# MoayedHajiAli/ElasticDiffusion-official

Hardware: AMD Instinct MI355X
Metric: images/sec at 50 steps (SDXL 2048x1024) (higher is better)
Workload: dtype fp16

## Files before the change

### elasticdiffusion_official_amd/_hip.py

```python
import ctypes
import os
import subprocess

import torch

PKG_DIR = os.path.dirname(os.path.abspath(__file__))
ROOT_DIR = os.path.dirname(PKG_DIR)
SOURCES = [os.path.join(PKG_DIR, "csrc", n) for n in ("elastic_kernels.hip", "unet_kernels.hip", "attention_kernels.hip", "gemm_kernels.hip", "vae_kernels.hip",
                                                       "canny_kernels.hip", "resize_kernels.hip", "mask_kernels.hip", "lora_kernels.hip", "pca_kernels.hip")]
SRC = SOURCES[0]
INCLUDE = os.path.join(ROOT_DIR, "include")
SO_PATH = os.path.join(PKG_DIR, "libelastic_hip.so")
ABI_VERSION = 13

HIPCC_FLAGS = ["--offload-arch=gfx950", "-O3", "-std=c++17", "-ffp-contract=off", "-fPIC", "-shared"]

_i32p = ctypes.POINTER(ctypes.c_int32)
_vp, _i, _f, _i64 = ctypes.c_void_p, ctypes.c_int, ctypes.c_float, ctypes.c_int64

SIGNATURES = {
    "ed_version": [],
    "ed_error_string": [_i],
    "ed_gather_views": [_vp, _vp, _i, _i, _i, _i, _i, _vp, _vp, _i, _i, _i, _i, _i, _i, _i, _vp, _f, _vp],
    "ed_scatter_centres": [_vp, _i, _vp, _i, _i, _i, _i, _i, _i, _i, _vp, _vp, _vp, _vp, _vp],
    "ed_pick_assemble": [_vp, _vp, _vp, _vp, _vp, _vp, _i, _vp, _i, _i, _i, _i, _i, _i, _i, _i, _i, _i, _i, _vp],
    "ed_unpad_direction": [_vp, _i, _vp, _vp, _i, _i, _i, _i, _i, _i, _i, _i, _i, _vp],
    "ed_fill_directions": [_vp, _vp, _vp, _vp, _vp, _vp, _vp, _vp, _vp, _vp, _i, _i, _i, _i, _i, _i, _i, _vp],
    "ed_cfg_ddim_step": [_vp, _vp, _vp, _vp, _vp, _f, _f, _f, _f, _f, _i64, _vp],
    "ed_undo_step": [_vp, _vp, _vp, _vp, _i, _i64, _vp],
    "ed_rrg_update": [_vp, _vp, _vp, _vp, _vp, _vp, _vp, _vp, _f, _f, _f, _f, _f, _i, _i, _i, _i, _i, _i, _vp],
    "ed_gather2d": [_vp, _i, _vp, _i, _i, _i, _i, _vp, _vp, _vp, _i, _i, _i, _vp],
    "ed_tile_gather_pad": [_vp, _vp, _i, _i, _i, _i, _i, _vp, _vp, _i, _i, _f, _vp],
    "ed_tile_accumulate_normalise": [_vp, _i, _vp, _i, _i, _i, _i, _i, _i, _vp, _vp, _vp, _vp, _vp],
    "ed_geglu": [_vp, _vp, _i, _i64, _i, _vp],
    "ed_groupnorm": [_vp, _vp, _vp, _vp, _vp, _vp, _vp, _i, _i, _i, _i, _i, _f, _i, _i, _vp],
    "ed_groupnorm_workspace": [_i, _i, _i, _i],
    "ed_bias_residual_add": [_vp, _vp, _vp, _vp, _vp, _i, _i, _i, _i, _i, _vp],
    "ed_add_layernorm": [_vp, _vp, _vp, _vp, _vp, _vp, _i, _i64, _i, _f, _vp],
    "ed_tokens_add_nchw": [_vp, _vp, _vp, _i, _i, _i, _i, _vp],
    "ed_layernorm": [_vp, _vp, _vp, _vp, _i, _i64, _i, _f, _vp],
    "ed_layernorm_s32": [_vp, _vp, _vp, _vp, _i, _i64, _i, _f, _vp],
    "ed_add_layernorm_s32": [_vp, _vp, _vp, _vp, _vp, _vp, _i, _i64, _i, _f, _vp],
    "ed_groupnorm_nhwc_s32": [_vp, _vp, _vp, _vp, _vp, _i, _i, _i, _i, _i, _f, _i, _vp],
    "ed_groupnorm_nhwc": [_vp, _vp, _vp, _vp, _vp, _vp, _vp, _i, _i, _i, _i, _i, _f, _i, _vp],
    "ed_groupnorm_nhwc_workspace": [_i, _i, _i, _i],
    "ed_groupnorm_nhwc_cat": [_vp, _vp, _vp, _vp, _vp, _vp, _i, _i, _i, _i, _i, _i, _f, _i, _vp],
    "ed_assemble_rows": [_vp, _i, _i, _i, _i, _vp, _vp, _vp, _vp, _vp, _vp, _i, _i, _i, _i, _i, _i, _i, _vp, _vp, _vp, _vp,
                         _i, _i, _i, _i, _i, _i, _i, _i, _vp],
# ... 66 lines not shown
    "ed_assemble_rows_n": [_vp, _i, _i, _i, _i, _vp, _vp, _vp, _vp, _vp, _vp, _i, _i, _i, _i, _i, _i, _i, _vp, _vp, _vp, _vp,
                           _i, _i, _i, _i, _i, _i, _i, _i, _vp, _i, _vp, _i, _vp],
    "ed_region_blend": [_vp, _vp, _vp, _i, _i, _i64, _vp],
    "ed_phase_epilogue_rg": [_vp, _vp, _i, _vp, _vp, _vp, _vp, _vp, _vp, _vp, _vp, _vp, _vp, _vp, _vp, _vp, _vp, _vp, _vp,
                             _vp, _vp, _vp, _vp, _i, _i, _i, _i, _i, _i, _i, _i, _i, _i, _i, _i, _i, _i, _f, _f, _f, _f, _f,
                             _f, _f, _f, _f, _i, _vp, _vp, _f, _f, _vp, _i, _vp, _i, _vp],
    "ed_phase_moments_rg": [_vp, _vp, _i, _vp, _vp, _vp, _vp, _vp, _vp, _vp, _vp, _vp, _vp, _vp, _vp, _vp, _vp, _i, _i, _i, _i,
                            _i, _i, _i, _i, _i, _i, _i, _i, _i, _i, _f, _vp, _i, _vp],
    "ed_score_pca_workspace": [_i, _i64],
    "ed_score_pca_fit": [_vp, _i, _i, _i, _i, _i, _vp, _vp, _vp, _vp, _vp, _vp],
    "ed_score_pca_map": [_vp, _i, _i, _i, _i, _vp, _vp, _vp, _vp],
    "ed_groupnorm_nhwc_f32_weighted": [_vp, _vp, _vp, _vp, _vp, _i, _i, _i, _i, _i, _f, _i, _i, _vp, _vp, _vp],
    "ed_groupnorm_f32_weighted": [_vp, _vp, _vp, _vp, _vp, _i, _i, _i, _i, _i, _f, _i, _vp, _vp, _vp],
    "ed_softmax_rows_bias": [_vp, _i64, _i64, _f, _vp, _vp],
    "ed_control_residuals": [_vp, _i, _i, _vp, _i64, _vp],
    "ed_flash_attention_ipn": [_vp, _vp, _vp, _vp, _i, _i, _i, _i, _i, _i, _vp, _i, _i64, _i64, _i64, _i64, _i64, _i64, _i64, _i64, _f,
                               _vp, _vp],
    "ed_flash_attention_ipm": [_vp, _vp, _vp, _vp, _i, _i, _i, _i, _i, _i, _vp, _i, _i64, _i64, _i64, _i64, _i64, _i64, _i64, _i64, _f,
                               _vp, _vp, _i64, _i64, _vp],
    "ed_ip_mask_rows": [_vp, _i, _i, _i, _i, _vp, _vp, _vp, _i, _i, _i, _i, _i, _vp, _vp, _i, _i, _i, _i, _i, _i, _i, _i, _vp, _vp],
}

_LIB = None


def build_library(force=False, verbose=False):
    deps = SOURCES + [os.path.join(INCLUDE, "elastic_hip.h")]
    if not force and os.path.isfile(SO_PATH) and os.path.getmtime(SO_PATH) >= max(os.path.getmtime(d) for d in deps):
        return SO_PATH
    import tempfile
    flags = [f for f in HIPCC_FLAGS if f != "-shared"]
    with tempfile.TemporaryDirectory(prefix="ed_build_") as tmp:
        objs = [os.path.join(tmp, os.path.basename(src) + ".o") for src in SOURCES]
        cmds = [["hipcc", *flags, "-I", INCLUDE, "-c", src, "-o", obj] for src, obj in zip(SOURCES, objs)]
        if verbose:
            for c in cmds:
                print(" ".join(c))
        procs = [subprocess.Popen(c) for c in cmds]
        codes = [p.wait() for p in procs]
        if any(codes):
            raise subprocess.CalledProcessError(next(c for c in codes if c), cmds[[bool(c) for c in codes].index(True)])
        link = ["hipcc", "--offload-arch=gfx950", "-fPIC", "-shared", *objs, "-o", SO_PATH + ".tmp"]
        if verbose:
            print(" ".join(link))
        subprocess.run(link, check=True)
        os.replace(SO_PATH + ".tmp", SO_PATH)
    return SO_PATH


def lib():
    global _LIB
    if _LIB is None:
        if not os.path.isfile(SO_PATH):
            raise RuntimeError(
                f"{SO_PATH} is missing: the HIP kernels are the product path and there is no CPU fallback. "
                "Build it with `python -c 'import __graft_entry__ as g; g.build()'`.")
        L = ctypes.CDLL(SO_PATH)
        for name, argtypes in SIGNATURES.items():
            fn = getattr(L, name)
            fn.argtypes = argtypes
            fn.restype = (ctypes.c_char_p if name == "ed_error_string" else
                          ctypes.c_int64 if name.endswith("_workspace") else ctypes.c_int)
        if L.ed_version() != ABI_VERSION:
            raise RuntimeError(f"libelastic_hip.so ABI {L.ed_version()} != expected {ABI_VERSION}; rebuild")
        _LIB = L
    return _LIB

# ... 6 lines not shown
```

### elasticdiffusion_official_amd/csrc/attention_kernels.hip

```cpp
#include <hip/hip_runtime.h>
#include <stdint.h>

#include "elastic_hip.h"

namespace {

constexpr int D = 64;
constexpr int QB = 128;
constexpr int KT = 64;
constexpr int K_LD = 72;
constexpr int V_LD_TR = 96;
constexpr int V_LD_T = 68;

typedef float f32x16 __attribute__((ext_vector_type(16)));
typedef float f32x8 __attribute__((ext_vector_type(8)));
typedef short s16x4 __attribute__((ext_vector_type(4)));
typedef short s16x8 __attribute__((ext_vector_type(8)));
typedef __bf16 bf16x8 __attribute__((ext_vector_type(8)));
typedef _Float16 f16x8 __attribute__((ext_vector_type(8)));

struct alignas(16) Vec16 { uint32_t w[4]; };
struct alignas(8) Vec8 { uint32_t w[2]; };

struct BF {
  typedef bf16x8 v8;
  static __device__ __forceinline__ f32x16 mfma(v8 a, v8 b, f32x16 c) {
    return __builtin_amdgcn_mfma_f32_32x32x16_bf16(a, b, c, 0, 0, 0);
  }
  static __device__ __forceinline__ v8 pack(f32x8 p) { return __builtin_convertvector(p, v8); }
};
struct HF {
  typedef f16x8 v8;
  static __device__ __forceinline__ f32x16 mfma(v8 a, v8 b, f32x16 c) {
    return __builtin_amdgcn_mfma_f32_32x32x16_f16(a, b, c, 0, 0, 0);
// ... 388 lines not shown
    pf[g] = T::pack(pv);
    asm volatile("" : "+v"(pf[g]));
  }
}

template <typename T>
__device__ __forceinline__ void resoftmax_tile(const uint16_t* kt, int ln, int hi, const typename T::v8 (&qf)[4],
                                               f32x16 (&s)[2], float sl, SoftmaxRun& r, typename T::v8 (&pf)[4]) {
  qk_tile<T>(kt, ln, hi, qf, s);
  float mx = s[0][0];
#pragma unroll
  for (int j = 1; j < 16; ++j) mx = fmaxf(mx, s[0][j]);
#pragma unroll
  for (int j = 0; j < 16; ++j) mx = fmaxf(mx, s[1][j]);
  mx = fmaxf(mx, __shfl_xor(mx, 32, 64));
  const float use = fmaxf(r.mb, mx * sl);
  r.alpha = __builtin_amdgcn_exp2f(r.mb - use);
  r.mb = use;
  float psum = 0.f;
#pragma unroll
  for (int g = 0; g < 4; ++g) {
    f32x8 pv;
#pragma unroll
    for (int j = 0; j < 8; ++j) {
      const int f = 8 * g + j;
      pv[j] = __builtin_amdgcn_exp2f(__builtin_fmaf(s[f >> 4][f & 15], sl, -use));
      psum += pv[j];
    }
    pf[g] = T::pack(pv);
  }
  r.psum = psum;
}

template <typename T, bool HAS_PV, bool HAS_NEXT, bool LAZY, bool EXP2, int DEPTH, class Filler>
__device__ __forceinline__ void pipe_region(Filler&& filler, const uint16_t* k_next, const uint16_t* v_prev, int lane, int ln, int hi,
                                            const typename T::v8 (&qf)[4], f32x16 (&s_cur)[2], f32x16 (&s_next)[2],
                                            const typename T::v8 (&p_prev)[4], typename T::v8 (&p_cur)[4],
                                            f32x16 (&o)[2], float sl, SoftmaxRun& run, const f32x16& negm) {
  constexpr int NQK = HAS_NEXT ? 8 : 0, N = NQK + (HAS_PV ? 8 : 0);
  auto fetch = [&](int i) -> Vec16 {
    if (i < NQK) return *reinterpret_cast<const Vec16*>(&k_next[(32 * (i & 1) + ln) * K_LD + 16 * (i >> 1) + 8 * hi]);
    const int j = i - NQK;
    return v_frag_tr(v_prev, lane, hi, j >> 1, j & 1);
  };
  if (HAS_NEXT && !EXP2) {
#pragma unroll
    for (int i = 0; i < 16; ++i) s_next[0][i] = s_next[1][i] = 0.f;
  }
  Vec16 ring[DEPTH + 1];
#pragma unroll
  for (int r = 0; r <= DEPTH; ++r) ring[r] = Vec16{{0u, 0u, 0u, 0u}};
#pragma unroll
  for (int r = 0; r < DEPTH; ++r)
    if (r < N) ring[r] = fetch(r);
#pragma unroll
  for (int i = 0; i < 16; ++i) {
    if (i < N) {
      if (i + DEPTH < N) ring[(i + DEPTH) % (DEPTH + 1)] = fetch(i + DEPTH);
      const Vec16 a_cur = ring[i % (DEPTH + 1)];
      if (i < NQK) {
        if (EXP2 && i < 2) s_next[i & 1] = T::mfma(as_v8<typename T::v8>(a_cur), qf[0], negm);
        else s_next[i & 1] = T::mfma(as_v8<typename T::v8>(a_cur), qf[i >> 1], s_next[i & 1]);
        asm volatile("" : "+v"(s_next[i & 1]));
      } else {
        const int j = i - NQK;
        o[j & 1] = T::mfma(as_v8<typename T::v8>(a_cur), p_prev[j >> 1], o[j & 1]);
        asm volatile("" : "+v"(o[j & 1]));
      }
    }
    if (LAZY) softmax_slice_lazy<T, EXP2>(i, s_cur, sl, run, p_cur);
    else softmax_slice<T>(i, s_cur, sl, run, p_cur);
    filler(i);
    __builtin_amdgcn_sched_barrier(0);
  }
}

template <typename T, bool LAZY, bool EXP2 = false, int DEPTH = 1, int WAVES = 4>
__global__ void __launch_bounds__(64 * WAVES, 2)
k_flash_attn_pipe(const Params p) {
  static_assert(LAZY || !EXP2, "the exponent-domain variant is built on the lazy-maximum loop");
  static_assert(WAVES == 4 || WAVES == 8, "4 or 8 waves per workgroup");
  constexpr int NK = LAZY ? 3 : 2;
  constexpr int NST = 8 / WAVES;
  __shared__ SmemPipe<NK> sm;
  const int tid = threadIdx.x;
  const int lane = tid & 63, wave = tid >> 6;
  const int ln = lane & 31, hi = lane >> 5;
  int bh, qblk;
  {
    const int id = blockIdx.x, per = 8 * p.nqb, grp = id / per, r = id - grp * per;
    if ((grp + 1) * 8 <= p.BH) {
      bh = grp * 8 + (r & 7);
      qblk = r >> 3;
    } else {
      bh = grp * 8 + r / p.nqb;
      qblk = r % p.nqb;
    }
  }
  const int b = bh / p.H, h = bh - b * p.H;
  const uint16_t* qg = p.q + b * p.q_sb + h * D;
  const uint16_t* kg = p.k + b * p.k_sb + h * D;
  const uint16_t* vg = p.v + b * p.v_sb + h * D;
  uint16_t* og = p.o + b * p.o_sb + h * D;

  const int q_row = qblk * (32 * WAVES) + wave * 32 + ln;
  typename T::v8 qf[4];
#pragma unroll
  for (int ks = 0; ks < 4; ++ks) qf[ks] = as_v8<typename T::v8>(load_row16(qg, p.q_sn, q_row, p.Nq, 16 * ks + 8 * hi));

  const BufRsrc k_rs = make_rsrc(kg, ((int64_t)(p.Nk - 1) * p.k_sn + D) * 2);
  const BufRsrc v_rs = make_rsrc(vg, ((int64_t)(p.Nk - 1) * p.v_sn + D) * 2);
  const int st_row = tid >> 3, st_col = (tid & 7) * 8;
  const uint32_t k_off = (uint32_t)(((int64_t)st_row * p.k_sn + st_col) * 2), k_half = (uint32_t)(32 * p.k_sn * 2);
  const uint32_t v_off = (uint32_t)(((int64_t)st_row * p.v_sn + st_col) * 2), v_half = (uint32_t)(32 * p.v_sn * 2);
  Vec16 kreg[NST], vreg[NST];
  auto load_k = [&](int t) {
    const uint32_t base = k_off + (uint32_t)t * 2u * k_half;
#pragma unroll
    for (int i = 0; i < NST; ++i) kreg[i] = buf_load16(k_rs, base + i * k_half, 0);
  };
  auto load_v = [&](int t) {
    const uint32_t base = v_off + (uint32_t)t * 2u * v_half;
#pragma unroll
    for (int i = 0; i < NST; ++i) vreg[i] = buf_load16(v_rs, base + i * v_half, 0);
  };
  auto write_k = [&](int buf) {
#pragma unroll
    for (int i = 0; i < NST; ++i) *reinterpret_cast<Vec16*>(&sm.k[buf][(st_row + 32 * i) * K_LD + st_col]) = kreg[i];
  };
  auto write_v = [&](int buf) {
#pragma unroll
    for (int i = 0; i < NST; ++i) *reinterpret_cast<Vec16*>(&sm.v[buf][(st_row + 32 * i) * V_LD_TR + st_col]) = vreg[i];
  };

  f32x16 oacc[2];
#pragma unroll
  for (int i = 0; i < 16; ++i) oacc[0][i] = oacc[1][i] = 0.f;
  SoftmaxRun run;
  run.mb = -INFINITY, run.l = 0.f, run.mx = 0.f, run.use = 0.f, run.alpha = 1.f, run.psum = 0.f;
  const float sl = EXP2 ? 1.0f : p.scale_log2e;
  const int n_tiles = (p.Nk + KT - 1) / KT, n_full = p.Nk / KT;
  f32x16 negm;
#pragma unroll
  for (int i = 0; i < 16; ++i) negm[i] = 0.f;

  load_k(0);
  load_v(0);
  Vec16 k1reg[NST];
#pragma unroll
  for (int i = 0; i < NST; ++i) k1reg[i] = buf_load16(k_rs, k_off + 2u * k_half + i * k_half, 0);
  write_k(0);
  write_v(0);
#pragma unroll
  for (int i = 0; i < NST; ++i) *reinterpret_cast<Vec16*>(&sm.k[1][(st_row + 32 * i) * K_LD + st_col]) = k1reg[i];
  __syncthreads();

  f32x16 sA[2], sB[2];
  typename T::v8 pA[4], pB[4];
  int vb_prev = 2, vb_cur = 0, vb_next = 1;
  int kb_cur = 0, kb_next = 1, kb_write = NK == 3 ? 2 : 0;

  auto iter = [&](auto has_pv, auto has_next, int t, f32x16 (&s_cur)[2], f32x16 (&s_next)[2],
                  typename T::v8 (&p_prev)[4], typename T::v8 (&p_cur)[4]) {
    const uint32_t kbase = k_off + (uint32_t)(t + 2) * 2u * k_half, vbase = v_off + (uint32_t)(t + 1) * 2u * v_half;
    uint16_t* const kdst = sm.k[kb_write];
    uint16_t* const vdst = sm.v[vb_next];
    auto filler = [&](int i) {
      if (i < NST) kreg[i] = buf_load16(k_rs, kbase + i * k_half, 0);
      else if (i < 2 * NST) vreg[i - NST] = buf_load16(v_rs, vbase + (i - NST) * v_half, 0);
      else if (i >= 11 && i < 11 + NST) *reinterpret_cast<Vec16*>(&kdst[(st_row + 32 * (i - 11)) * K_LD + st_col]) = kreg[i - 11];
      else if (i >= 11 + NST && i < 11 + 2 * NST)
        *reinterpret_cast<Vec16*>(&vdst[(st_row + 32 * (i - 11 - NST)) * V_LD_TR + st_col]) = vreg[i - 11 - NST];
    };
    constexpr bool lazy = LAZY && (EXP2 || decltype(has_pv)::value);
    pipe_region<T, decltype(has_pv)::value, decltype(has_next)::value, lazy, EXP2, DEPTH>(filler, sm.k[kb_next], sm.v[vb_prev], lane, ln,
                                                                                          hi, qf, s_cur, s_next, p_prev, p_cur,
                                                                                          oacc, sl, run, negm);
    if (lazy) {
      run.alpha = 1.0f;
      if (__any(!(run.psum <= RESCALE_SUM_MAX))) {
        const float mb_old = run.mb;
        resoftmax_tile<T>(sm.k[kb_cur], ln, hi, qf, s_cur, sl, run, p_cur);
        if (EXP2) {
          const float d = run.mb - mb_old;
          if (decltype(has_next)::value) {
#pragma unroll
            for (int i = 0; i < 16; ++i) s_next[0][i] -= d, s_next[1][i] -= d;
          }
#pragma unroll
          for (int i = 0; i < 16; ++i) negm[i] = -run.mb;
          asm volatile("" : "+v"(negm));
        }
      }
      run.l = __builtin_fmaf(run.l, run.alpha, run.psum);
    }
    if (__any(run.alpha != 1.0f)) {
#pragma unroll
      for (int i = 0; i < 16; ++i) {
        oacc[0][i] *= run.alpha;
        oacc[1][i] *= run.alpha;
      }
    }
    const int tmp = vb_prev;
    vb_prev = vb_cur, vb_cur = vb_next, vb_next = tmp;
    const int ktmp = kb_cur;
    kb_cur = kb_next, kb_next = kb_write, kb_write = NK == 3 ? ktmp : kb_cur;
    __syncthreads();
  };

  if (n_full > 0) {
    qk_tile<T>(sm.k[0], ln, hi, qf, sA);
    if (EXP2) {
      float mx = sA[0][0];
#pragma unroll
      for (int j = 1; j < 16; ++j) mx = fmaxf(mx, sA[0][j]);
#pragma unroll
      for (int j = 0; j < 16; ++j) mx = fmaxf(mx, sA[1][j]);
      mx = fmaxf(mx, __shfl_xor(mx, 32, 64));
      run.mb = mx;
#pragma unroll
      for (int i = 0; i < 16; ++i) sA[0][i] -= mx, sA[1][i] -= mx, negm[i] = -mx;
      asm volatile("" : "+v"(negm));
    }
    __syncthreads();
    if (n_full == 1) {
      iter(False{}, False{}, 0, sA, sB, pB, pA);
    } else {
      iter(False{}, True{}, 0, sA, sB, pB, pA);
      int t = 1;
      for (; t + 2 < n_full; t += 2) {
        iter(True{}, True{}, t, sB, sA, pA, pB);
        iter(True{}, True{}, t + 1, sA, sB, pB, pA);
      }
      if (n_full - t == 2) {
        iter(True{}, True{}, t, sB, sA, pA, pB);
        iter(True{}, False{}, t + 1, sA, sB, pB, pA);
      } else {
        iter(True{}, False{}, t, sB, sA, pA, pB);
      }
    }
    if ((n_full - 1) & 1) pv_tile<T>(sm.v[vb_prev], lane, hi, pB, oacc);
    else pv_tile<T>(sm.v[vb_prev], lane, hi, pA, oacc);
  }

  if (n_tiles > n_full) {
    f32x16 s[2];
    qk_tile<T>(sm.k[kb_cur], ln, hi, qf, s);
#pragma unroll
    for (int kb = 0; kb < 2; ++kb)
#pragma unroll
      for (int r = 0; r < 16; ++r)
        if (n_full * KT + 32 * kb + 8 * (r >> 2) + 4 * hi + (r & 3) >= p.Nk) s[kb][r] = -INFINITY;
    float mx = s[0][0];
#pragma unroll
    for (int r = 1; r < 16; ++r) mx = fmaxf(mx, s[0][r]);
#pragma unroll
    for (int r = 0; r < 16; ++r) mx = fmaxf(mx, s[1][r]);
    mx = fmaxf(mx, __shfl_xor(mx, 32, 64));
    const float use = fmaxf(run.mb, mx * sl);
    const float alpha = __builtin_amdgcn_exp2f(run.mb - use);
    float psum = 0.f;
#pragma unroll
    for (int kb = 0; kb < 2; ++kb)
#pragma unroll
      for (int r = 0; r < 16; ++r) {
        const float e = __builtin_amdgcn_exp2f(__builtin_fmaf(s[kb][r], sl, -use));
        s[kb][r] = e;
        psum += e;
      }
    run.l = __builtin_fmaf(run.l, alpha, psum);
#pragma unroll
    for (int i = 0; i < 16; ++i) {
      oacc[0][i] *= alpha;
      oacc[1][i] *= alpha;
    }
    typename T::v8 pf[4];
#pragma unroll
    for (int st = 0; st < 4; ++st) {
      f32x8 pv;
#pragma unroll
      for (int j = 0; j < 8; ++j) pv[j] = s[st >> 1][8 * (st & 1) + j];
      pf[st] = T::pack(pv);
    }
    pv_tile<T>(sm.v[vb_cur], lane, hi, pf, oacc);
  }

  const float l_tot = run.l + __shfl_xor(run.l, 32, 64);
  const float inv = 1.0f / l_tot;
  store_o_row<T>(og + (int64_t)q_row * p.o_sn, oacc, inv, hi, q_row < p.Nq);
}

constexpr int SK_QBLOCKS = 4;

template <int NKB>
struct SmemSmall {
  uint16_t k[32 * NKB * K_LD];
  uint16_t v[32 * NKB * V_LD_TR];
};

template <typename T, int NKB>
__global__ void __launch_bounds__(256, 2)
k_flash_attn_smallkv(const Params p) {
  __shared__ SmemSmall<NKB> sm;
  const int tid = threadIdx.x;
  const int lane = tid & 63, wave = tid >> 6;
  const int ln = lane & 31, hi = lane >> 5;
  const int nqg = p.nqb;
  const int bh = blockIdx.x / nqg, qgrp = blockIdx.x - bh * nqg;
  const int b = bh / p.H, h = bh - b * p.H;
  const uint16_t* qg = p.q + b * p.q_sb + h * D;
  const uint16_t* kg = p.k + b * p.k_sb + h * D;
  const uint16_t* vg = p.v + b * p.v_sb + h * D;
  uint16_t* og = p.o + b * p.o_sb + h * D;

  for (int idx = tid; idx < 32 * NKB * 8; idx += 256) {
    const int row = idx >> 3, col = (idx & 7) * 8;
    *reinterpret_cast<Vec16*>(&sm.k[row * K_LD + col]) = load_row16(kg, p.k_sn, row, p.Nk, col);
    *reinterpret_cast<Vec16*>(&sm.v[row * V_LD_TR + col]) = load_row16(vg, p.v_sn, row, p.Nk, col);
  }
  __syncthreads();
  const float sl = p.scale_log2e;

// ... 628 lines not shown
        s[kb][r] = e;
        psum += e;
      }
    l_run = __builtin_fmaf(l_run, alpha, psum);
#pragma unroll
    for (int db = 0; db < G::NDB; ++db)
#pragma unroll
      for (int i = 0; i < 16; ++i) oacc[db][i] *= alpha;

#pragma unroll
    for (int st = 0; st < 4; ++st) {
      f32x8 pv;
#pragma unroll
      for (int j = 0; j < 8; ++j) pv[j] = s[st >> 1][8 * (st & 1) + j];
      const typename T::v8 pf = T::pack(pv);
#pragma unroll
      for (int db = 0; db < G::NDB; ++db) {
        const int row = 16 * st + 4 * hi + ((lane & 15) >> 2);
        const int col = 32 * db + 16 * ((lane >> 4) & 1) + 4 * (lane & 3);
        typedef s16x4 __attribute__((address_space(3))) * lds_s16x4_ptr;
        const s16x4 lo = __builtin_amdgcn_ds_read_tr16_b64_v4i16((lds_s16x4_ptr)(&sm.v[buf][row * G::VLD + col]));
        const s16x4 hi4 = __builtin_amdgcn_ds_read_tr16_b64_v4i16((lds_s16x4_ptr)(&sm.v[buf][(row + 8) * G::VLD + col]));
        const Vec16 vf = __builtin_bit_cast(Vec16, __builtin_shufflevector(lo, hi4, 0, 1, 2, 3, 4, 5, 6, 7));
        oacc[db] = T::mfma(as_v8<typename T::v8>(vf), pf, oacc[db]);
      }
    }
    if (t + 1 < n_tiles) write_lds(buf ^ 1);
    __syncthreads();
  }

  const float l_tot = l_run + __shfl_xor(l_run, 32, 64);
  const float inv = 1.0f / l_tot;
  store_o_row<T, G::NDB>(og + (int64_t)q_row * p.o_sn, oacc, inv, hi, q_row < p.Nq, DH);
}

}

extern "C" {

int ed_flash_attention(const void* q, const void* k, const void* v, void* out, int dtype, int B, int H, int Nq, int Nk,
                       int head_dim, int64_t q_sb, int64_t q_sn, int64_t k_sb, int64_t k_sn, int64_t v_sb, int64_t v_sn,
                       int64_t o_sb, int64_t o_sn, float scale, int v_path, void* stream) {
  if (B == 0 || H == 0 || Nq == 0) return 0;
  if (Nk <= 0) return (int)hipErrorInvalidValue;
  if (head_dim != D) {
    if (head_dim != 40 && head_dim != 80 && head_dim != 160) return (int)hipErrorInvalidValue;
    if (dtype != ED_BF16 && dtype != ED_F16) return (int)hipErrorInvalidValue;
    if ((((uintptr_t)q | (uintptr_t)k | (uintptr_t)v) & 15u) || ((uintptr_t)out & 7u)) return (int)hipErrorInvalidValue;
    if ((q_sb | q_sn | k_sb | k_sn | v_sb | v_sn) % 8 || (o_sb | o_sn) % 4) return (int)hipErrorInvalidValue;
    Params p;
    p.q = (const uint16_t*)q, p.k = (const uint16_t*)k, p.v = (const uint16_t*)v, p.o = (uint16_t*)out;
    p.Nq = Nq, p.Nk = Nk, p.H = H, p.BH = B * H, p.nqb = (Nq + QB - 1) / QB;
    p.q_sb = q_sb, p.q_sn = q_sn, p.k_sb = k_sb, p.k_sn = k_sn, p.v_sb = v_sb, p.v_sn = v_sn, p.o_sb = o_sb, p.o_sn = o_sn;
    p.scale_log2e = scale * 1.44269504088896340736f;
    const int64_t nb = (int64_t)p.BH * p.nqb;
    if (nb > 0x7fffffff) return (int)hipErrorInvalidValue;
    const dim3 grid((unsigned)nb), block(256);
    hipStream_t st = (hipStream_t)stream;
#define ED_FG(DHV)                                                                      \
  if (dtype == ED_BF16) k_flash_attn_gen<BF, DHV><<<grid, block, 0, st>>>(p);           \
  else k_flash_attn_gen<HF, DHV><<<grid, block, 0, st>>>(p);
    if (head_dim == 40) { ED_FG(40) } else if (head_dim == 80) { ED_FG(80) } else { ED_FG(160) }
#undef ED_FG
    return (int)hipGetLastError();
  }
  if ((((uintptr_t)q | (uintptr_t)k | (uintptr_t)v) & 15u) || ((uintptr_t)out & 7u)) return (int)hipErrorInvalidValue;
  if ((q_sb | q_sn | k_sb | k_sn | v_sb | v_sn) % 8 || (o_sb | o_sn) % 4) return (int)hipErrorInvalidValue;
  Params p;
  p.q = (const uint16_t*)q, p.k = (const uint16_t*)k, p.v = (const uint16_t*)v, p.o = (uint16_t*)out;
  hipStream_t st = (hipStream_t)stream;
  if ((v_path >= 4 && v_path <= 10)) {
    if (v_path == 8 && Nk > 160) return (int)hipErrorInvalidValue;
    if ((v_path == 6 || v_path == 7 || v_path == 9 || v_path == 10) && Nk < 64) return (int)hipErrorInvalidValue;
    if (v_path != 8 && ((int64_t)(Nk + 2 * KT) * (k_sn > v_sn ? k_sn : v_sn) * 2 >= 0x7fffffffll)) return (int)hipErrorInvalidValue;
    const int rows_per_wg = v_path == 8 ? QB * SK_QBLOCKS : (v_path >= 9 ? 2 * QB : QB);
    p.Nq = Nq, p.Nk = Nk, p.H = H, p.BH = B * H, p.nqb = (Nq + rows_per_wg - 1) / rows_per_wg;
    p.q_sb = q_sb, p.q_sn = q_sn, p.k_sb = k_sb, p.k_sn = k_sn, p.v_sb = v_sb, p.v_sn = v_sn, p.o_sb = o_sb, p.o_sn = o_sn;
    p.scale_log2e = scale * 1.44269504088896340736f;
    const int64_t nb = (int64_t)p.BH * p.nqb;
    if (nb > 0x7fffffff) return (int)hipErrorInvalidValue;
    const dim3 grid((unsigned)nb), block(256);
    if (dtype != ED_BF16 && dtype != ED_F16) return (int)hipErrorInvalidValue;
    if (v_path == 4) {
      if (dtype == ED_BF16) k_flash_attn_pipe<BF, false><<<grid, block, 0, st>>>(p);
      else k_flash_attn_pipe<HF, false><<<grid, block, 0, st>>>(p);
    } else if (v_path == 5) {
      if (dtype == ED_BF16) k_flash_attn_pipe<BF, true><<<grid, block, 0, st>>>(p);
      else k_flash_attn_pipe<HF, true><<<grid, block, 0, st>>>(p);
    } else if (v_path == 6) {
      if (dtype == ED_BF16) k_flash_attn_pipe<BF, true, true><<<grid, block, 0, st>>>(p);
      else k_flash_attn_pipe<HF, true, true><<<grid, block, 0, st>>>(p);
    } else if (v_path == 7) {
      if (dtype == ED_BF16) k_flash_attn_pipe<BF, false, false, 3><<<grid, block, 0, st>>>(p);
      else k_flash_attn_pipe<HF, false, false, 3><<<grid, block, 0, st>>>(p);
    } else if (v_path == 9) {
      if (dtype == ED_BF16) k_flash_attn_pipe<BF, false, false, 1, 8><<<grid, dim3(512), 0, st>>>(p);
      else k_flash_attn_pipe<HF, false, false, 1, 8><<<grid, dim3(512), 0, st>>>(p);
    } else if (v_path == 10) {
      if (dtype == ED_BF16) k_flash_attn_pipe<BF, true, false, 1, 8><<<grid, dim3(512), 0, st>>>(p);
      else k_flash_attn_pipe<HF, true, false, 1, 8><<<grid, dim3(512), 0, st>>>(p);
    } else if (Nk <= 64) {
      if (dtype == ED_BF16) k_flash_attn_smallkv<BF, 2><<<grid, block, 0, st>>>(p);
      else k_flash_attn_smallkv<HF, 2><<<grid, block, 0, st>>>(p);
    } else if (Nk <= 96) {
      if (dtype == ED_BF16) k_flash_attn_smallkv<BF, 3><<<grid, block, 0, st>>>(p);
      else k_flash_attn_smallkv<HF, 3><<<grid, block, 0, st>>>(p);
    } else {
      if (dtype == ED_BF16) k_flash_attn_smallkv<BF, 5><<<grid, block, 0, st>>>(p);
      else k_flash_attn_smallkv<HF, 5><<<grid, block, 0, st>>>(p);
    }
    return (int)hipGetLastError();
  }
  const int qn = (v_path & 2) ? 2 : 1;
  p.Nq = Nq, p.Nk = Nk, p.H = H, p.BH = B * H, p.nqb = (Nq + QB * qn - 1) / (QB * qn);
  p.q_sb = q_sb, p.q_sn = q_sn, p.k_sb = k_sb, p.k_sn = k_sn, p.v_sb = v_sb, p.v_sn = v_sn, p.o_sb = o_sb, p.o_sn = o_sn;
  p.scale_log2e = scale * 1.44269504088896340736f;
  const int64_t blocks = (int64_t)p.BH * p.nqb;
  if (blocks > 0x7fffffff) return (int)hipErrorInvalidValue;
// ... 124 lines not shown
```

### elasticdiffusion_official_amd/ops.py

```python
import ctypes
import math

import torch

from . import _hip

ED_F32, ED_F16, ED_BF16 = 0, 1, 2
_DTYPE = {torch.float32: ED_F32, torch.float16: ED_F16, torch.bfloat16: ED_BF16}


_LAUNCH = {"device": None}


def _stream_of(t):
    if _LAUNCH["device"] is None:
        _LAUNCH["device"] = t.device
    return _stream()


def _stream():
    dev = _LAUNCH["device"]
    if dev is None:
        raise RuntimeError("internal: _stream() before any device tensor argument")
    return torch.cuda.current_stream(dev).cuda_stream
# ... 1274 lines not shown
FLASH_HEAD_DIMS = (40, 64, 80, 160)
FLASH_EXP2 = False
_ENV_VARIANT = __import__("os").environ.get("ED_FLASH_VARIANT")
LOG2E = 1.4426950408889634


def _pipe_fits(Nk, row_stride):
    return Nk >= 128 and (Nk + 128) * row_stride * 2 < 2 ** 31


def flash_prescale(Nq, Nk, row_stride, scale=0.125):
    if FLASH_V_PATH is not None:
        want = int(FLASH_V_PATH)
    elif _ENV_VARIANT is not None:
        want = -1 if _ENV_VARIANT == "legacy" else int(_ENV_VARIANT)
    else:
        want = 6 if FLASH_EXP2 else -1
    return scale * LOG2E if (want == 6 and _pipe_fits(Nk, row_stride)) else None


def _flash_variant(B, heads, Nq, Nk, k=None, v=None, prescaled=False):
    fits = k is None or _pipe_fits(Nk, max(k.stride(1), v.stride(1)))
    if prescaled:
        if not (Nk >= 128 and fits):
            _reject("flash_attention: exponent-domain q needs the pipelined kernel (Nk >= 128, 32-bit K / V offsets)")
        return 6
    if FLASH_V_PATH is not None and int(FLASH_V_PATH) != 6:
        return int(FLASH_V_PATH)
    legacy = 2 if (Nq >= 2048 and Nk >= 1024 and B * heads * (Nq // 256) >= 1024) else 0
    if _ENV_VARIANT == "legacy":
        return legacy
    if _ENV_VARIANT is not None and int(_ENV_VARIANT) != 6:
        want = int(_ENV_VARIANT)
        if want in (4, 5, 7, 9, 10):
            return want if (Nk >= 128 and fits) else (8 if Nk <= 96 else legacy)
        return want if (want != 8 or Nk <= SMALLKV_MAX_KEYS) else legacy
    if Nk <= 96 or _stream_two_chunks(Nq, Nk):
        return 8
    if Nk >= 128 and fits:
        return FLASH_DEFAULT_PIPE
    return legacy


SMALLKV_MAX_KEYS = 160


def _stream_two_chunks(Nq, Nk):
    return 128 <= Nk <= SMALLKV_MAX_KEYS and Nq >= 4096


FLASH_DEFAULT_PIPE = 5


def flash_attention(q, k, v, heads, v_path=None, prescaled=False):
    B, Nq, HD = q.shape
    Nk = k.shape[1]
    hd = HD // heads
    if HD != heads * hd or hd not in FLASH_HEAD_DIMS or k.shape != (B, Nk, HD) or v.shape != (B, Nk, HD):
        _reject(f"flash_attention: head_dim must be one of {FLASH_HEAD_DIMS} and shapes consistent (q {tuple(q.shape)}, "
                f"k {tuple(k.shape)}, v {tuple(v.shape)}, heads {heads})")
    if hd != 64 and (prescaled or v_path is not None):
        _reject("flash_attention: kernel variants exist for head_dim 64 only")
    for t, name in ((q, "q"), (k, "k"), (v, "v")):
        if not t.is_cuda or t.dtype != q.dtype or t.stride(2) != 1:
            _reject(f"flash_attention: {name} must be a 16-bit tensor on the MI355X with unit last stride; no CPU fallback")
        if _LAUNCH["device"] is None:
            _LAUNCH["device"] = t.device
        elif _LAUNCH["device"] != t.device:
            _reject(f"flash_attention: {name} lives on {t.device}, q on {_LAUNCH['device']}")
    if v_path is not None and (int(v_path) == 6) != bool(prescaled):
        _reject("flash_attention: v_path 6 takes exponent-domain q (prescaled=True) and nothing else does")
    out = torch.empty(B, Nq, HD, dtype=q.dtype, device=q.device)
    TIMER.note_work("ed_flash_attention", flops=4.0 * B * heads * Nq * Nk * hd,
                    nbytes=2.0 * q.element_size() * HD * B * (Nq + Nk))
# ... 679 lines not shown
```

Measured before the change: 0.1075.

## Add 64-rows-per-wave flash attention variant and MFMA VGPR-form compile flag

Adds an opt-in variant of the pipelined flash attention kernel in which each wave processes two 32-row query slices. Both slices share the K/V fragment loads from LDS, and the V loads come first in the pipeline. The variant is chosen only through path 11 or an environment variable, because the selector heuristic returns false. Separately, attention_kernels.hip is now built with an LLVM flag that makes MFMA use VGPR-form accumulators, which can change register allocation and code generation for all attention kernels, including the default ones.

After: 0.1076 (median of 2 runs). About the same (+0.1%).

```diff
diff --git a/elasticdiffusion_official_amd/_hip.py b/elasticdiffusion_official_amd/_hip.py
--- a/elasticdiffusion_official_amd/_hip.py
+++ b/elasticdiffusion_official_amd/_hip.py
@@ -14,6 +14,7 @@
 ABI_VERSION = 13
 
 HIPCC_FLAGS = ["--offload-arch=gfx950", "-O3", "-std=c++17", "-ffp-contract=off", "-fPIC", "-shared"]
+EXTRA_FLAGS = {"attention_kernels.hip": ["-mllvm", "-amdgpu-mfma-vgpr-form"]}
 
 _i32p = ctypes.POINTER(ctypes.c_int32)
 _vp, _i, _f, _i64 = ctypes.c_void_p, ctypes.c_int, ctypes.c_float, ctypes.c_int64
@@ -146,7 +147,8 @@
     flags = [f for f in HIPCC_FLAGS if f != "-shared"]
     with tempfile.TemporaryDirectory(prefix="ed_build_") as tmp:
         objs = [os.path.join(tmp, os.path.basename(src) + ".o") for src in SOURCES]
-        cmds = [["hipcc", *flags, "-I", INCLUDE, "-c", src, "-o", obj] for src, obj in zip(SOURCES, objs)]
+        cmds = [["hipcc", *flags, *EXTRA_FLAGS.get(os.path.basename(src), []), "-I", INCLUDE, "-c", src, "-o", obj]
+                for src, obj in zip(SOURCES, objs)]
         if verbose:
             for c in cmds:
                 print(" ".join(c))
diff --git a/elasticdiffusion_official_amd/csrc/attention_kernels.hip b/elasticdiffusion_official_amd/csrc/attention_kernels.hip
--- a/elasticdiffusion_official_amd/csrc/attention_kernels.hip
+++ b/elasticdiffusion_official_amd/csrc/attention_kernels.hip
@@ -1,5 +1,6 @@
 #include <hip/hip_runtime.h>
 #include <stdint.h>
+#include <stdlib.h>
 
 #include "elastic_hip.h"
 
@@ -454,20 +455,26 @@
   r.psum = psum;
 }
 
-template <typename T, bool HAS_PV, bool HAS_NEXT, bool LAZY, bool EXP2, int DEPTH, class Filler>
+template <typename T, bool HAS_PV, bool HAS_NEXT, bool LAZY, bool EXP2, int DEPTH, int QN, class Filler>
 __device__ __forceinline__ void pipe_region(Filler&& filler, const uint16_t* k_next, const uint16_t* v_prev, int lane, int ln, int hi,
-                                            const typename T::v8 (&qf)[4], f32x16 (&s_cur)[2], f32x16 (&s_next)[2],
-                                            const typename T::v8 (&p_prev)[4], typename T::v8 (&p_cur)[4],
-                                            f32x16 (&o)[2], float sl, SoftmaxRun& run, const f32x16& negm) {
-  constexpr int NQK = HAS_NEXT ? 8 : 0, N = NQK + (HAS_PV ? 8 : 0);
+                                            const typename T::v8 (&qf)[QN][4], f32x16 (&s_cur)[QN][2], f32x16 (&s_next)[QN][2],
+                                            const typename T::v8 (&p_prev)[QN][4], typename T::v8 (&p_cur)[QN][4],
+                                            f32x16 (&o)[QN][2], float sl, SoftmaxRun (&run)[QN], const f32x16& negm) {
+  constexpr int NQK = HAS_NEXT ? 8 : 0, NPV = HAS_PV ? 8 : 0, N = NQK + NPV;
+  constexpr int QK0 = QN == 2 ? NPV : 0, PV0 = QN == 2 ? 0 : NQK;
   auto fetch = [&](int i) -> Vec16 {
-    if (i < NQK) return *reinterpret_cast<const Vec16*>(&k_next[(32 * (i & 1) + ln) * K_LD + 16 * (i >> 1) + 8 * hi]);
-    const int j = i - NQK;
+    if (i >= QK0 && i < QK0 + NQK) {
+      const int j = i - QK0;
+      return *reinterpret_cast<const Vec16*>(&k_next[(32 * (j & 1) + ln) * K_LD + 16 * (j >> 1) + 8 * hi]);
+    }
+    const int j = i - PV0;
     return v_frag_tr(v_prev, lane, hi, j >> 1, j & 1);
   };
   if (HAS_NEXT && !EXP2) {
 #pragma unroll
-    for (int i = 0; i < 16; ++i) s_next[0][i] = s_next[1][i] = 0.f;
+    for (int qn = 0; qn < QN; ++qn)
+#pragma unroll
+      for (int i = 0; i < 16; ++i) s_next[qn][0][i] = s_next[qn][1][i] = 0.f;
   }
   Vec16 ring[DEPTH + 1];
 #pragma unroll
@@ -477,31 +484,39 @@
     if (r < N) ring[r] = fetch(r);
 #pragma unroll
   for (int i = 0; i < 16; ++i) {
+    Vec16 a_cur = Vec16{{0u, 0u, 0u, 0u}};
     if (i < N) {
       if (i + DEPTH < N) ring[(i + DEPTH) % (DEPTH + 1)] = fetch(i + DEPTH);
-      const Vec16 a_cur = ring[i % (DEPTH + 1)];
-      if (i < NQK) {
-        if (EXP2 && i < 2) s_next[i & 1] = T::mfma(as_v8<typename T::v8>(a_cur), qf[0], negm);
-        else s_next[i & 1] = T::mfma(as_v8<typename T::v8>(a_cur), qf[i >> 1], s_next[i & 1]);
-        asm volatile("" : "+v"(s_next[i & 1]));
-      } else {
-        const int j = i - NQK;
-        o[j & 1] = T::mfma(as_v8<typename T::v8>(a_cur), p_prev[j >> 1], o[j & 1]);
-        asm volatile("" : "+v"(o[j & 1]));
-      }
-    }
-    if (LAZY) softmax_slice_lazy<T, EXP2>(i, s_cur, sl, run, p_cur);
-    else softmax_slice<T>(i, s_cur, sl, run, p_cur);
-    filler(i);
-    __builtin_amdgcn_sched_barrier(0);
-  }
-}
-
-template <typename T, bool LAZY, bool EXP2 = false, int DEPTH = 1, int WAVES = 4>
-__global__ void __launch_bounds__(64 * WAVES, 2)
+      a_cur = ring[i % (DEPTH + 1)];
+    }
+#pragma unroll
+    for (int qn = 0; qn < QN; ++qn) {
+      if (i < N) {
+        if (i >= QK0 && i < QK0 + NQK) {
+          const int j = i - QK0;
+          if (EXP2 && j < 2) s_next[qn][j & 1] = T::mfma(as_v8<typename T::v8>(a_cur), qf[qn][0], negm);
+          else s_next[qn][j & 1] = T::mfma(as_v8<typename T::v8>(a_cur), qf[qn][j >> 1], s_next[qn][j & 1]);
+          asm volatile("" : "+v"(s_next[qn][j & 1]));
+        } else {
+          const int j = i - PV0;
+          o[qn][j & 1] = T::mfma(as_v8<typename T::v8>(a_cur), p_prev[qn][j >> 1], o[qn][j & 1]);
+          asm volatile("" : "+v"(o[qn][j & 1]));
+        }
+      }
+      if (LAZY) softmax_slice_lazy<T, EXP2>(i, s_cur[qn], sl, run[qn], p_cur[qn]);
+      else softmax_slice<T>(i, s_cur[qn], sl, run[qn], p_cur[qn]);
+      if (qn == 0) filler(i);
+      __builtin_amdgcn_sched_barrier(0);
+    }
+  }
+}
+
+template <typename T, bool LAZY, bool EXP2 = false, int DEPTH = 1, int WAVES = 4, int QN = 1>
+__global__ void __launch_bounds__(64 * WAVES, QN == 1 ? 2 : 1)
 k_flash_attn_pipe(const Params p) {
   static_assert(LAZY || !EXP2, "the exponent-domain variant is built on the lazy-maximum loop");
   static_assert(WAVES == 4 || WAVES == 8, "4 or 8 waves per workgroup");
+  static_assert(QN == 1 || (QN == 2 && WAVES == 4 && LAZY && !EXP2), "64 rows per wave: 4 waves, lazy maximum, natural-domain q");
   constexpr int NK = LAZY ? 3 : 2;
   constexpr int NST = 8 / WAVES;
   __shared__ SmemPipe<NK> sm;
@@ -525,10 +540,13 @@
   const uint16_t* vg = p.v + b * p.v_sb + h * D;
   uint16_t* og = p.o + b * p.o_sb + h * D;
 
-  const int q_row = qblk * (32 * WAVES) + wave * 32 + ln;
-  typename T::v8 qf[4];
-#pragma unroll
-  for (int ks = 0; ks < 4; ++ks) qf[ks] = as_v8<typename T::v8>(load_row16(qg, p.q_sn, q_row, p.Nq, 16 * ks + 8 * hi));
+  const int q_row = qblk * (32 * WAVES * QN) + wave * (32 * QN) + ln;
+  typename T::v8 qf[QN][4];
+#pragma unroll
+  for (int qn = 0; qn < QN; ++qn)
+#pragma unroll
+    for (int ks = 0; ks < 4; ++ks)
+      qf[qn][ks] = as_v8<typename T::v8>(load_row16(qg, p.q_sn, q_row + 32 * qn, p.Nq, 16 * ks + 8 * hi));
 
   const BufRsrc k_rs = make_rsrc(kg, ((int64_t)(p.Nk - 1) * p.k_sn + D) * 2);
   const BufRsrc v_rs = make_rsrc(vg, ((int64_t)(p.Nk - 1) * p.v_sn + D) * 2);
@@ -555,11 +573,14 @@
     for (int i = 0; i < NST; ++i) *reinterpret_cast<Vec16*>(&sm.v[buf][(st_row + 32 * i) * V_LD_TR + st_col]) = vreg[i];
   };
 
-  f32x16 oacc[2];
-#pragma unroll
-  for (int i = 0; i < 16; ++i) oacc[0][i] = oacc[1][i] = 0.f;
-  SoftmaxRun run;
-  run.mb = -INFINITY, run.l = 0.f, run.mx = 0.f, run.use = 0.f, run.alpha = 1.f, run.psum = 0.f;
+  f32x16 oacc[QN][2];
+  SoftmaxRun run[QN];
+#pragma unroll
+  for (int qn = 0; qn < QN; ++qn) {
+#pragma unroll
+    for (int i = 0; i < 16; ++i) oacc[qn][0][i] = oacc[qn][1][i] = 0.f;
+    run[qn].mb = -INFINITY, run[qn].l = 0.f, run[qn].mx = 0.f, run[qn].use = 0.f, run[qn].alpha = 1.f, run[qn].psum = 0.f;
+  }
   const float sl = EXP2 ? 1.0f : p.scale_log2e;
   const int n_tiles = (p.Nk + KT - 1) / KT, n_full = p.Nk / KT;
   f32x16 negm;
@@ -577,13 +598,14 @@
   for (int i = 0; i < NST; ++i) *reinterpret_cast<Vec16*>(&sm.k[1][(st_row + 32 * i) * K_LD + st_col]) = k1reg[i];
   __syncthreads();
 
-  f32x16 sA[2], sB[2];
-  typename T::v8 pA[4], pB[4];
+  f32x16 sA[QN][2], sB[QN][2];
+  typename T::v8 pA[QN][4], pB_[QN][4];
+  typename T::v8 (&pB)[QN][4] = QN == 2 ? pA : pB_;
   int vb_prev = 2, vb_cur = 0, vb_next = 1;
   int kb_cur = 0, kb_next = 1, kb_write = NK == 3 ? 2 : 0;
 
-  auto iter = [&](auto has_pv, auto has_next, int t, f32x16 (&s_cur)[2], f32x16 (&s_next)[2],
-                  typename T::v8 (&p_prev)[4], typename T::v8 (&p_cur)[4]) {
+  auto iter = [&](auto has_pv, auto has_next, int t, f32x16 (&s_cur)[QN][2], f32x16 (&s_next)[QN][2],
+                  typename T::v8 (&p_prev)[QN][4], typename T::v8 (&p_cur)[QN][4]) {
     const uint32_t kbase = k_off + (uint32_t)(t + 2) * 2u * k_half, vbase = v_off + (uint32_t)(t + 1) * 2u * v_half;
     uint16_t* const kdst = sm.k[kb_write];
     uint16_t* const vdst = sm.v[vb_next];
@@ -595,32 +617,35 @@
         *reinterpret_cast<Vec16*>(&vdst[(st_row + 32 * (i - 11 - NST)) * V_LD_TR + st_col]) = vreg[i - 11 - NST];
     };
     constexpr bool lazy = LAZY && (EXP2 || decltype(has_pv)::value);
-    pipe_region<T, decltype(has_pv)::value, decltype(has_next)::value, lazy, EXP2, DEPTH>(filler, sm.k[kb_next], sm.v[vb_prev], lane, ln,
-                                                                                          hi, qf, s_cur, s_next, p_prev, p_cur,
-                                                                                          oacc, sl, run, negm);
-    if (lazy) {
-      run.alpha = 1.0f;
-      if (__any(!(run.psum <= RESCALE_SUM_MAX))) {
-        const float mb_old = run.mb;
-        resoftmax_tile<T>(sm.k[kb_cur], ln, hi, qf, s_cur, sl, run, p_cur);
-        if (EXP2) {
-          const float d = run.mb - mb_old;
-          if (decltype(has_next)::value) {
-#pragma unroll
-            for (int i = 0; i < 16; ++i) s_next[0][i] -= d, s_next[1][i] -= d;
+    pipe_region<T, decltype(has_pv)::value, decltype(has_next)::value, lazy, EXP2, DEPTH, QN>(filler, sm.k[kb_next], sm.v[vb_prev], lane,
+                                                                                              ln, hi, qf, s_cur, s_next, p_prev, p_cur,
+                                                                                              oacc, sl, run, negm);
+#pragma unroll
+    for (int qn = 0; qn < QN; ++qn) {
+      if (lazy) {
+        run[qn].alpha = 1.0f;
+        if (__any(!(run[qn].psum <= RESCALE_SUM_MAX))) {
+          const float mb_old = run[qn].mb;
+          resoftmax_tile<T>(sm.k[kb_cur], ln, hi, qf[qn], s_cur[qn], sl, run[qn], p_cur[qn]);
+          if (EXP2) {
+            const float d = run[qn].mb - mb_old;
+            if (decltype(has_next)::value) {
+#pragma unroll
+              for (int i = 0; i < 16; ++i) s_next[qn][0][i] -= d, s_next[qn][1][i] -= d;
+            }
+#pragma unroll
+            for (int i = 0; i < 16; ++i) negm[i] = -run[qn].mb;
+            asm volatile("" : "+v"(negm));
           }
-#pragma unroll
-          for (int i = 0; i < 16; ++i) negm[i] = -run.mb;
-          asm volatile("" : "+v"(negm));
         }
-      }
-      run.l = __builtin_fmaf(run.l, run.alpha, run.psum);
-    }
-    if (__any(run.alpha != 1.0f)) {
-#pragma unroll
-      for (int i = 0; i < 16; ++i) {
-        oacc[0][i] *= run.alpha;
-        oacc[1][i] *= run.alpha;
+        run[qn].l = __builtin_fmaf(run[qn].l, run[qn].alpha, run[qn].psum);
+      }
+      if (__any(run[qn].alpha != 1.0f)) {
+#pragma unroll
+        for (int i = 0; i < 16; ++i) {
+          oacc[qn][0][i] *= run[qn].alpha;
+          oacc[qn][1][i] *= run[qn].alpha;
+        }
       }
     }
     const int tmp = vb_prev;
@@ -631,17 +656,18 @@
   };
 
   if (n_full > 0) {
-    qk_tile<T>(sm.k[0], ln, hi, qf, sA);
+#pragma unroll
+    for (int qn = 0; qn < QN; ++qn) qk_tile<T>(sm.k[0], ln, hi, qf[qn], sA[qn]);
     if (EXP2) {
-      float mx = sA[0][0];
-#pragma unroll
-      for (int j = 1; j < 16; ++j) mx = fmaxf(mx, sA[0][j]);
-#pragma unroll
-      for (int j = 0; j < 16; ++j) mx = fmaxf(mx, sA[1][j]);
+      float mx = sA[0][0][0];
+#pragma unroll
+      for (int j = 1; j < 16; ++j) mx = fmaxf(mx, sA[0][0][j]);
+#pragma unroll
+      for (int j = 0; j < 16; ++j) mx = fmaxf(mx, sA[0][1][j]);
       mx = fmaxf(mx, __shfl_xor(mx, 32, 64));
-      run.mb = mx;
-#pragma unroll
-      for (int i = 0; i < 16; ++i) sA[0][i] -= mx, sA[1][i] -= mx, negm[i] = -mx;
+      run[0].mb = mx;
+#pragma unroll
+      for (int i = 0; i < 16; ++i) sA[0][0][i] -= mx, sA[0][1][i] -= mx, negm[i] = -mx;
       asm volatile("" : "+v"(negm));
     }
     __syncthreads();
@@ -661,55 +687,64 @@
         iter(True{}, False{}, t, sB, sA, pA, pB);
       }
     }
-    if ((n_full - 1) & 1) pv_tile<T>(sm.v[vb_prev], lane, hi, pB, oacc);
-    else pv_tile<T>(sm.v[vb_prev], lane, hi, pA, oacc);
+#pragma unroll
+    for (int qn = 0; qn < QN; ++qn) {
+      if ((n_full - 1) & 1) pv_tile<T>(sm.v[vb_prev], lane, hi, pB[qn], oacc[qn]);
+      else pv_tile<T>(sm.v[vb_prev], lane, hi, pA[qn], oacc[qn]);
+    }
   }
 
   if (n_tiles > n_full) {
-    f32x16 s[2];
-    qk_tile<T>(sm.k[kb_cur], ln, hi, qf, s);
-#pragma unroll
-    for (int kb = 0; kb < 2; ++kb)
-#pragma unroll
-      for (int r = 0; r < 16; ++r)
-        if (n_full * KT + 32 * kb + 8 * (r >> 2) + 4 * hi + (r & 3) >= p.Nk) s[kb][r] = -INFINITY;
-    float mx = s[0][0];
-#pragma unroll
-    for (int r = 1; r < 16; ++r) mx = fmaxf(mx, s[0][r]);
-#pragma unroll
-    for (int r = 0; r < 16; ++r) mx = fmaxf(mx, s[1][r]);
-    mx = fmaxf(mx, __shfl_xor(mx, 32, 64));
-    const float use = fmaxf(run.mb, mx * sl);
-    const float alpha = __builtin_amdgcn_exp2f(run.mb - use);
-    float psum = 0.f;
-#pragma unroll
-    for (int kb = 0; kb < 2; ++kb)
-#pragma unroll
-      for (int r = 0; r < 16; ++r) {
-        const float e = __builtin_amdgcn_exp2f(__builtin_fmaf(s[kb][r], sl, -use));
-        s[kb][r] = e;
-        psum += e;
-      }
-    run.l = __builtin_fmaf(run.l, alpha, psum);
-#pragma unroll
-    for (int i = 0; i < 16; ++i) {
-      oacc[0][i] *= alpha;
-      oacc[1][i] *= alpha;
-    }
-    typename T::v8 pf[4];
-#pragma unroll
-    for (int st = 0; st < 4; ++st) {
-      f32x8 pv;
-#pragma unroll
-      for (int j = 0; j < 8; ++j) pv[j] = s[st >> 1][8 * (st & 1) + j];
-      pf[st] = T::pack(pv);
-    }
-    pv_tile<T>(sm.v[vb_cur], lane, hi, pf, oacc);
-  }
-
-  const float l_tot = run.l + __shfl_xor(run.l, 32, 64);
-  const float inv = 1.0f / l_tot;
-  store_o_row<T>(og + (int64_t)q_row * p.o_sn, oacc, inv, hi, q_row < p.Nq);
+#pragma unroll
+    for (int qn = 0; qn < QN; ++qn) {
+      f32x16 s[2];
+      qk_tile<T>(sm.k[kb_cur], ln, hi, qf[qn], s);
+#pragma unroll
+      for (int kb = 0; kb < 2; ++kb)
+#pragma unroll
+        for (int r = 0; r < 16; ++r)
+          if (n_full * KT + 32 * kb + 8 * (r >> 2) + 4 * hi + (r & 3) >= p.Nk) s[kb][r] = -INFINITY;
+      float mx = s[0][0];
+#pragma unroll
+      for (int r = 1; r < 16; ++r) mx = fmaxf(mx, s[0][r]);
+#pragma unroll
+      for (int r = 0; r < 16; ++r) mx = fmaxf(mx, s[1][r]);
+      mx = fmaxf(mx, __shfl_xor(mx, 32, 64));
+      const float use = fmaxf(run[qn].mb, mx * sl);
+      const float alpha = __builtin_amdgcn_exp2f(run[qn].mb - use);
+      float psum = 0.f;
+#pragma unroll
+      for (int kb = 0; kb < 2; ++kb)
+#pragma unroll
+        for (int r = 0; r < 16; ++r) {
+          const float e = __builtin_amdgcn_exp2f(__builtin_fmaf(s[kb][r], sl, -use));
+          s[kb][r] = e;
+          psum += e;
+        }
+      run[qn].l = __builtin_fmaf(run[qn].l, alpha, psum);
+#pragma unroll
+      for (int i = 0; i < 16; ++i) {
+        oacc[qn][0][i] *= alpha;
+        oacc[qn][1][i] *= alpha;
+      }
+      typename T::v8 pf[4];
+#pragma unroll
+      for (int st = 0; st < 4; ++st) {
+        f32x8 pv;
+#pragma unroll
+        for (int j = 0; j < 8; ++j) pv[j] = s[st >> 1][8 * (st & 1) + j];
+        pf[st] = T::pack(pv);
+      }
+      pv_tile<T>(sm.v[vb_cur], lane, hi, pf, oacc[qn]);
+    }
+  }
+
+#pragma unroll
+  for (int qn = 0; qn < QN; ++qn) {
+    const float l_tot = run[qn].l + __shfl_xor(run[qn].l, 32, 64);
+    const float inv = 1.0f / l_tot;
+    store_o_row<T>(og + (int64_t)(q_row + 32 * qn) * p.o_sn, oacc[qn], inv, hi, q_row + 32 * qn < p.Nq);
+  }
 }
 
 constexpr int SK_QBLOCKS = 4;
@@ -1404,6 +1439,13 @@
   const float l_tot = l_run + __shfl_xor(l_run, 32, 64);
   const float inv = 1.0f / l_tot;
   store_o_row<T, G::NDB>(og + (int64_t)q_row * p.o_sn, oacc, inv, hi, q_row < p.Nq, DH);
+}
+
+constexpr int ROWS64_DEPTH = 1;
+
+inline bool flash_rows64_wins(int64_t BH, int Nq, int Nk) {
+  (void)BH, (void)Nq, (void)Nk;
+  return false;
 }
 
 }
@@ -1441,11 +1483,20 @@
   Params p;
   p.q = (const uint16_t*)q, p.k = (const uint16_t*)k, p.v = (const uint16_t*)v, p.o = (uint16_t*)out;
   hipStream_t st = (hipStream_t)stream;
+  bool rows64 = false;
+  if (v_path == 11 || v_path == 12) {
+    if (v_path == 11 && Nk < KT) return (int)hipErrorInvalidValue;
+    rows64 = v_path == 11;
+    v_path = 5;
+  } else if (v_path == 5) {
+    rows64 = flash_rows64_wins((int64_t)B * H, Nq, Nk);
+    if (const char* e = getenv("ED_FLASH_ROWS64")) rows64 = e[0] == '1' ? Nk >= KT : (e[0] == '0' ? false : rows64);
+  }
   if ((v_path >= 4 && v_path <= 10)) {
     if (v_path == 8 && Nk > 160) return (int)hipErrorInvalidValue;
     if ((v_path == 6 || v_path == 7 || v_path == 9 || v_path == 10) && Nk < 64) return (int)hipErrorInvalidValue;
     if (v_path != 8 && ((int64_t)(Nk + 2 * KT) * (k_sn > v_sn ? k_sn : v_sn) * 2 >= 0x7fffffffll)) return (int)hipErrorInvalidValue;
-    const int rows_per_wg = v_path == 8 ? QB * SK_QBLOCKS : (v_path >= 9 ? 2 * QB : QB);
+    const int rows_per_wg = v_path == 8 ? QB * SK_QBLOCKS : ((v_path >= 9 || rows64) ? 2 * QB : QB);
     p.Nq = Nq, p.Nk = Nk, p.H = H, p.BH = B * H, p.nqb = (Nq + rows_per_wg - 1) / rows_per_wg;
     p.q_sb = q_sb, p.q_sn = q_sn, p.k_sb = k_sb, p.k_sn = k_sn, p.v_sb = v_sb, p.v_sn = v_sn, p.o_sb = o_sb, p.o_sn = o_sn;
     p.scale_log2e = scale * 1.44269504088896340736f;
@@ -1456,6 +1507,9 @@
     if (v_path == 4) {
       if (dtype == ED_BF16) k_flash_attn_pipe<BF, false><<<grid, block, 0, st>>>(p);
       else k_flash_attn_pipe<HF, false><<<grid, block, 0, st>>>(p);
+    } else if (v_path == 5 && rows64) {
+      if (dtype == ED_BF16) k_flash_attn_pipe<BF, true, false, ROWS64_DEPTH, 4, 2><<<grid, block, 0, st>>>(p);
+      else k_flash_attn_pipe<HF, true, false, ROWS64_DEPTH, 4, 2><<<grid, block, 0, st>>>(p);
     } else if (v_path == 5) {
       if (dtype == ED_BF16) k_flash_attn_pipe<BF, true><<<grid, block, 0, st>>>(p);
       else k_flash_attn_pipe<HF, true><<<grid, block, 0, st>>>(p);
diff --git a/elasticdiffusion_official_amd/ops.py b/elasticdiffusion_official_amd/ops.py
--- a/elasticdiffusion_official_amd/ops.py
+++ b/elasticdiffusion_official_amd/ops.py
@@ -1330,7 +1330,7 @@
         return legacy
     if _ENV_VARIANT is not None and int(_ENV_VARIANT) != 6:
         want = int(_ENV_VARIANT)
-        if want in (4, 5, 7, 9, 10):
+        if want in (4, 5, 7, 9, 10, 11, 12):
             return want if (Nk >= 128 and fits) else (8 if Nk <= 96 else legacy)
         return want if (want != 8 or Nk <= SMALLKV_MAX_KEYS) else legacy
     if Nk <= 96 or _stream_two_chunks(Nq, Nk):
@@ -1338,6 +1338,10 @@
     if Nk >= 128 and fits:
         return FLASH_DEFAULT_PIPE
     return legacy
+
+
+def flash_rows64(BH, Nq, Nk):
+    return False
 
 
 SMALLKV_MAX_KEYS = 160
```
